# KTH-RPL/HiMo

Hardware: AMD Instinct MI355X
Metric: lidar_frames_per_sec_120k (higher is better)
Workload: dtype f16x2 (two-term split fp16, x = h + l with exact subnormals, on the matrix cores; float32 accumulate; ~22-bit products); 1 GPU; per-frame pipeline: pillarise 3 sweeps (512x512 grid) -> SeFlow++-style encoder/decoder + GRU head (random-init, self-specified: reference network source absent) -> per-point flow -> ego-motion removal + dt0 + flow2compDis -> comp_dis; points_per_frame=120000, sweeps_per_frame=3, parallelism=frames sharded x1, refined_output=False, batches_in_flight=3, matrix_arithmetic=f16x2, samples_per_backbone_launch=16, collectives=none (single process)

## Files before the change

### himo_amd/csrc/gruhead.hip

```cpp
#include "conv_common.h"
#include "bf16x3.h"

namespace himo {

struct GruHeadArgs {
    int64_t n;
    const int* pid; const float* offsets;
    const float* img0; const float* img1; int img_pitch;
    const float* dec; int dec_pitch;
    const float* w_off; const float* b_off;
    const unsigned short* wzr; const float* bzr;
    const unsigned short* wq; const float* bq;
    const unsigned short* w1; const float* b1;
    const float* w2; const float* b2;
    const float* xyz_t; const float* pts; int stride;
    float* flow;
    int iters;
    int img_split;
    unsigned* nonfinite;
    int w2_pitch;
};

constexpr int kGhMaxIters = 4;
struct GruHeadSave {
// ... 8 lines not shown
constexpr int kGhMaxSamples = 16;
struct GruHeadSample {
    int64_t n;
    const int* pid; const float* offsets; const float* img0; const float* img1; const float* dec;
    const float* xyz_t; const float* pts; float* flow; int stride;
};
struct GruHeadBatch {
    int n_samples;
    int block_start[kGhMaxSamples + 1];
    GruHeadSample s[kGhMaxSamples];
};

constexpr int kGhRows = 64;
constexpr bool kGhLaunder = false;

template <int SLABS>
__device__ inline int a_slot(int s, int slab, int row, int half) {
    return ((s * SLABS + slab) * kGhRows + row) * 32 + ((half ^ ((row >> 4) & 1)) << 4);
}

template <int FMT, int SLABS>
__device__ inline void a_store(unsigned char* A, int row, int k, float v) {
    constexpr int kGhPlane = SLABS * kGhRows * 32;
    unsigned h, m = 0, l;
    if (FMT == 3) split3(v, h, m, l); else split2(v, h, l);
    const int slab = k >> 4, kk = k & 15;
    const int off = a_slot<SLABS>(0, slab, row, kk >> 3) + (kk & 7) * 2;
    *reinterpret_cast<unsigned short*>(A + off) = (unsigned short)h;
    if (FMT == 3) *reinterpret_cast<unsigned short*>(A + off + kGhPlane) = (unsigned short)m;
    *reinterpret_cast<unsigned short*>(A + off + (FMT - 1) * kGhPlane) = (unsigned short)l;
// ... 44 lines not shown
#pragma unroll
        for (int rt = 0; rt < RT; ++rt)
#pragma unroll
            for (int t = 0; t < NT; ++t)
#pragma unroll
                for (int r = 0; r < 16; ++r)
                    acc[rt][t][r] = acc[rt][t][r] * kF16AccScale;
    }
}

template <int GROUP>
__device__ inline void sv_store(float* base, unsigned byte_off, float v) {
    *reinterpret_cast<float*>(reinterpret_cast<char*>(base) + byte_off) = v;
}

template <int FMT, int SLABS, bool SAVE = false>
__global__ __launch_bounds__(256, (FMT == 2 && !SAVE) ? 3 : 2) void gru_head_kernel(GruHeadArgs a, GruHeadBatch batch, GruHeadSave sv) {
    constexpr bool FOLD = SLABS == 9;
    static_assert(!(SAVE && FOLD), "the training forward keeps x explicit");
    constexpr int kGhPlane = SLABS * kGhRows * 32;
    __shared__ __attribute__((aligned(16))) unsigned char A[FMT * kGhPlane];
    __shared__ int s_pid[kGhRows];
    const int wave = __builtin_amdgcn_readfirstlane(threadIdx.x >> 6), lane = threadIdx.x & 63;
    const int li = lane & 31, lh = lane >> 5;
    int bid = blockIdx.x;
    {
        int smp = 0;
        while (smp + 1 < batch.n_samples && bid >= batch.block_start[smp + 1]) ++smp;
        bid -= batch.block_start[smp];
        const GruHeadSample& g = batch.s[smp];
        a.n = g.n; a.pid = g.pid; a.offsets = g.offsets; a.img0 = g.img0; a.img1 = g.img1; a.dec = g.dec;
        a.xyz_t = g.xyz_t; a.pts = g.pts; a.flow = g.flow; a.stride = g.stride;
    }
    const int64_t r0 = (int64_t)bid * kGhRows;

    if (threadIdx.x < kGhRows) {
        const int64_t i = r0 + threadIdx.x;
        s_pid[threadIdx.x] = i < a.n ? a.pid[i] : -1;
    }
    if constexpr (FOLD) {
        const int row = threadIdx.x >> 2, q = threadIdx.x & 3;
        const int64_t i = r0 + row;
        float v[4] = {0.f, 0.f, 0.f, 0.f};
        if (q == 0) {
            if (i < a.n) { v[0] = a.offsets[i * 3]; v[1] = a.offsets[i * 3 + 1]; v[2] = a.offsets[i * 3 + 2]; }
            v[3] = 1.f;
        }
// ... 16 lines not shown
        }
    } else {
        const int row = threadIdx.x >> 2, q = threadIdx.x & 3;
        const int64_t i = r0 + row;
        float o0 = 0.f, o1 = 0.f, o2 = 0.f;
        if (i < a.n) { o0 = a.offsets[i * 3]; o1 = a.offsets[i * 3 + 1]; o2 = a.offsets[i * 3 + 2]; }
#pragma unroll
        for (int k = 0; k < 16; ++k) {
            const int c = q * 16 + k;
            const float v = fmaf(o2, a.w_off[128 + c], fmaf(o1, a.w_off[64 + c], o0 * a.w_off[c])) + a.b_off[c];
            a_store<FMT, SLABS>(A, row, 128 + c, v);
        }
    }
    __syncthreads();

    const float* src = wave == 0 ? a.img0 : wave == 1 ? a.img1 : a.dec + (wave - 2) * 32;
    const int src_pitch = wave < 2 ? a.img_pitch : a.dec_pitch;
    float h[2][16];
    {
        int cell[2][16];
#pragma unroll
        for (int rt = 0; rt < 2; ++rt)
#pragma unroll
            for (int r = 0; r < 16; ++r) cell[rt][r] = s_pid[rt * 32 + (r & 3) + 8 * (r >> 2) + 4 * lh];
        if (FMT == 2 && wave < 2 && a.img_split) {
            unsigned short hh[2][16], ll[2][16];
#pragma unroll
            for (int rt = 0; rt < 2; ++rt)
#pragma unroll
                for (int r = 0; r < 16; ++r) {
                    const unsigned short* rec = reinterpret_cast<const unsigned short*>(src + (int64_t)max(cell[rt][r], 0) * src_pitch + (li & ~15));
                    hh[rt][r] = rec[li & 15]; ll[rt][r] = rec[16 + (li & 15)];
                }
#pragma unroll
            for (int rt = 0; rt < 2; ++rt)
#pragma unroll
                for (int r = 0; r < 16; ++r)
                    h[rt][r] = cell[rt][r] >= 0 ? (float)__builtin_bit_cast(_Float16, hh[rt][r]) + (float)__builtin_bit_cast(_Float16, ll[rt][r]) : 0.f;
        } else {
#pragma unroll
// ... 140 lines not shown
            }
            a.flow[i * 3 + c] = out;
            if (a.nonfinite && !(fabsf(out) <= 3.4028234664e38f)) atomicOr(a.nonfinite, 1u);
        }
    }
}

}

using namespace himo;

static int gru_head_launch(int n_samples, const himo_head_sample* h_samples, int img_pitch, int dec_pitch,
                           const float* d_w_off, const float* d_b_off, bool folded,
                           const void* d_wzr_packed, const float* d_bzr, const void* d_wq_packed, const float* d_bq,
                           const void* d_w1_packed, const float* d_b1, const float* d_w2, const float* d_b2,
                           int iters, int packed_format, int img_split, unsigned* d_nonfinite, void* stream) {
    if (img_split && (packed_format != 1 || (img_pitch & 15))) return HIMO_ERR_INVALID_ARGUMENT;
    if (n_samples < 0 || n_samples > kGhMaxSamples || (n_samples && !h_samples)) return HIMO_ERR_INVALID_ARGUMENT;
    if (iters < 0 || !(packed_format == 0 || packed_format == 1) || img_pitch < 32 || dec_pitch < 64) return HIMO_ERR_INVALID_ARGUMENT;
    if ((!folded && (!d_w_off || !d_b_off)) || !d_wzr_packed || !d_bzr || !d_wq_packed || !d_bq || !d_w1_packed || !d_b1 || !d_w2 || !d_b2)
        return HIMO_ERR_INVALID_ARGUMENT;
    if ((reinterpret_cast<uintptr_t>(d_wzr_packed) | reinterpret_cast<uintptr_t>(d_wq_packed) | reinterpret_cast<uintptr_t>(d_w1_packed)) & 15)
        return HIMO_ERR_INVALID_ARGUMENT;
    GruHeadBatch b{};
    int64_t blocks = 0;
    for (int i = 0; i < n_samples; ++i) {
        const himo_head_sample& h = h_samples[i];
        if (h.n < 0 || h.pc_stride < 3) return HIMO_ERR_INVALID_ARGUMENT;
        if (h.n == 0) continue;
        if (!h.d_pid || !h.d_offsets || !h.d_img0 || !h.d_img1 || !h.d_dec || !h.d_xyz_t || !h.d_pts || !h.d_flow) return HIMO_ERR_INVALID_ARGUMENT;
        GruHeadSample& g = b.s[b.n_samples];
        g.n = h.n; g.pid = h.d_pid; g.offsets = h.d_offsets; g.img0 = h.d_img0; g.img1 = h.d_img1; g.dec = h.d_dec;
        g.xyz_t = h.d_xyz_t; g.pts = h.d_pts; g.flow = h.d_flow; g.stride = h.pc_stride;
        b.block_start[b.n_samples] = (int)blocks;
        blocks += (h.n + kGhRows - 1) / kGhRows;
        if (blocks > 0x7fffffff) return HIMO_ERR_INVALID_ARGUMENT;
        b.block_start[++b.n_samples] = (int)blocks;
    }
    if (!blocks) return HIMO_OK;
    GruHeadArgs a{};
    a.img_pitch = img_pitch; a.dec_pitch = dec_pitch; a.w_off = d_w_off; a.b_off = d_b_off;
    a.wzr = (const unsigned short*)d_wzr_packed; a.bzr = d_bzr; a.wq = (const unsigned short*)d_wq_packed; a.bq = d_bq;
    a.w1 = (const unsigned short*)d_w1_packed; a.b1 = d_b1; a.w2 = d_w2; a.b2 = d_b2; a.iters = iters;
    a.img_split = img_split ? 1 : 0;
    a.nonfinite = d_nonfinite;
    a.w2_pitch = 3;
    hipStream_t s = (hipStream_t)stream;
    ProfScope ps("gru_head_kernel", s);
    const dim3 grid((unsigned)blocks);
    const GruHeadSave none{};
    if (folded) {
        if (packed_format == 1) hipLaunchKernelGGL((gru_head_kernel<2, 9>), grid, dim3(256), 0, s, a, b, none);
        else hipLaunchKernelGGL((gru_head_kernel<3, 9>), grid, dim3(256), 0, s, a, b, none);
    } else {
        if (packed_format == 1) hipLaunchKernelGGL((gru_head_kernel<2, 12>), grid, dim3(256), 0, s, a, b, none);
        else hipLaunchKernelGGL((gru_head_kernel<3, 12>), grid, dim3(256), 0, s, a, b, none);
    }
    HIMO_LAUNCH_CHECK("gru_head_kernel");
    return HIMO_OK;
}

extern "C" int himo_gru_head_batch(int n_samples, const himo_head_sample* h_samples, int img_pitch, int dec_pitch,
                                   const float* d_w_off, const float* d_b_off,
                                   const void* d_wzr_packed, const float* d_bzr, const void* d_wq_packed, const float* d_bq,
                                   const void* d_w1_packed, const float* d_b1, const float* d_w2, const float* d_b2,
                                   int iters, int packed_format, int img_split, void* stream) {
    return gru_head_launch(n_samples, h_samples, img_pitch, dec_pitch, d_w_off, d_b_off, false, d_wzr_packed, d_bzr, d_wq_packed, d_bq,
                           d_w1_packed, d_b1, d_w2, d_b2, iters, packed_format, img_split, nullptr, stream);
}

extern "C" int himo_gru_head_batch_folded(int n_samples, const himo_head_sample* h_samples, int img_pitch, int dec_pitch,
                                          const void* d_wzr_packed, const float* d_bzr, const void* d_wq_packed, const float* d_bq,
                                          const void* d_w1_packed, const float* d_b1, const float* d_w2, const float* d_b2,
                                          int iters, int packed_format, int img_split, void* stream) {
    return gru_head_launch(n_samples, h_samples, img_pitch, dec_pitch, nullptr, nullptr, true, d_wzr_packed, d_bzr, d_wq_packed, d_bq,
                           d_w1_packed, d_b1, d_w2, d_b2, iters, packed_format, img_split, nullptr, stream);
}

extern "C" int himo_gru_head_batch_guarded(int n_samples, const himo_head_sample* h_samples, int img_pitch, int dec_pitch,
                                           const float* d_w_off, const float* d_b_off,
                                           const void* d_wzr_packed, const float* d_bzr, const void* d_wq_packed, const float* d_bq,
                                           const void* d_w1_packed, const float* d_b1, const float* d_w2, const float* d_b2,
                                           int iters, int packed_format, int img_split, uint32_t* d_nonfinite, void* stream) {
    if ((d_w_off == nullptr) != (d_b_off == nullptr)) return HIMO_ERR_INVALID_ARGUMENT;
    return gru_head_launch(n_samples, h_samples, img_pitch, dec_pitch, d_w_off, d_b_off, d_w_off == nullptr, d_wzr_packed, d_bzr, d_wq_packed,
                           d_bq, d_w1_packed, d_b1, d_w2, d_b2, iters, packed_format, img_split, d_nonfinite, stream);
}

extern "C" int himo_gru_head_train(int64_t n, const int32_t* d_pid, const float* d_offsets, const float* d_img0, const float* d_img1,
                                   int img_pitch, const float* d_dec, int dec_pitch, const float* d_w_off, const float* d_b_off,
                                   const void* d_wzr_packed, const float* d_bzr, const void* d_wq_packed, const float* d_bq,
                                   const void* d_w1_packed, const float* d_b1, const float* d_w2, int w2_pitch, const float* d_b2,
                                   int iters, int packed_format, const himo_head_saved* h_saved, uint32_t* d_nonfinite, void* stream) {
    if (n < 0 || iters < 1 || iters > kGhMaxIters || !(packed_format == 0 || packed_format == 1) || img_pitch < 32 || dec_pitch < 64 ||
        !(w2_pitch == 3 || w2_pitch == 4) || !h_saved)
        return HIMO_ERR_INVALID_ARGUMENT;
    if (!d_w_off || !d_b_off || !d_wzr_packed || !d_bzr || !d_wq_packed || !d_bq || !d_w1_packed || !d_b1 || !d_w2 || !d_b2)
        return HIMO_ERR_INVALID_ARGUMENT;
    if ((reinterpret_cast<uintptr_t>(d_wzr_packed) | reinterpret_cast<uintptr_t>(d_wq_packed) | reinterpret_cast<uintptr_t>(d_w1_packed)) & 15)
        return HIMO_ERR_INVALID_ARGUMENT;
    if (n == 0) return HIMO_OK;
// ... 7 lines not shown
        return HIMO_ERR_INVALID_ARGUMENT;
    GruHeadBatch b{};
    b.n_samples = 1;
    GruHeadSample& g = b.s[0];
    g.n = n; g.pid = d_pid; g.offsets = d_offsets; g.img0 = d_img0; g.img1 = d_img1; g.dec = d_dec;
    const int64_t blocks = (n + kGhRows - 1) / kGhRows;
    if (blocks > 0x7fffffff) return HIMO_ERR_INVALID_ARGUMENT;
    b.block_start[0] = 0; b.block_start[1] = (int)blocks;
    GruHeadArgs a{};
    a.img_pitch = img_pitch; a.dec_pitch = dec_pitch; a.w_off = d_w_off; a.b_off = d_b_off;
    a.wzr = (const unsigned short*)d_wzr_packed; a.bzr = d_bzr; a.wq = (const unsigned short*)d_wq_packed; a.bq = d_bq;
    a.w1 = (const unsigned short*)d_w1_packed; a.b1 = d_b1; a.w2 = d_w2; a.b2 = d_b2; a.iters = iters; a.w2_pitch = w2_pitch;
    a.nonfinite = d_nonfinite;
    hipStream_t s = (hipStream_t)stream;
    ProfScope ps("gru_head_train_kernel", s);
    if (packed_format == 1) hipLaunchKernelGGL((gru_head_kernel<2, 12, true>), dim3((unsigned)blocks), dim3(256), 0, s, a, b, sv);
    else hipLaunchKernelGGL((gru_head_kernel<3, 12, true>), dim3((unsigned)blocks), dim3(256), 0, s, a, b, sv);
    HIMO_LAUNCH_CHECK("gru_head_kernel<train>");
    return HIMO_OK;
}

extern "C" int himo_clear_u32(uint32_t* d_words, int n, void* stream) {
    if (!d_words || n < 1) return HIMO_ERR_INVALID_ARGUMENT;
    HIMO_HIP(hipMemsetAsync(d_words, 0, (size_t)n * 4, (hipStream_t)stream));
    return HIMO_OK;
}

extern "C" int himo_gru_head(int64_t n, const int32_t* d_pid, const float* d_offsets, const float* d_img0, const float* d_img1,
                             int img_pitch, const float* d_dec, int dec_pitch, const float* d_w_off, const float* d_b_off,
                             const void* d_wzr_packed, const float* d_bzr, const void* d_wq_packed, const float* d_bq,
                             const void* d_w1_packed, const float* d_b1, const float* d_w2, const float* d_b2,
                             const float* d_xyz_t, const float* d_pts, int pc_stride, float* d_flow, int iters, int packed_format,
// ... 6 lines not shown
```

### himo_amd/seflow/model.py

```python
from __future__ import annotations

import ctypes

import numpy as np
import torch

from .. import _lib
from . import spec

EPI_BIAS, EPI_BIAS_BN_GELU, EPI_BIAS_GELU, EPI_GRU_ZR, EPI_GRU_Q = range(5)


class ConvDesc(ctypes.Structure):
    _fields_ = [("x", ctypes.c_void_p), ("x_batch_stride", ctypes.c_int64), ("x_pitch", ctypes.c_int),
                ("w", ctypes.c_void_p), ("bias", ctypes.c_void_p), ("scale", ctypes.c_void_p), ("shift", ctypes.c_void_p),
                ("y", ctypes.c_void_p), ("y_batch_stride", ctypes.c_int64), ("y_pitch", ctypes.c_int),
                ("n", ctypes.c_int), ("h", ctypes.c_int), ("w_in", ctypes.c_int), ("cin", ctypes.c_int),
                ("cout", ctypes.c_int), ("ksize", ctypes.c_int), ("stride", ctypes.c_int), ("epilogue", ctypes.c_int),
                ("aux_in", ctypes.c_void_p), ("aux_in_pitch", ctypes.c_int),
                ("aux_out", ctypes.c_void_p), ("aux_out_pitch", ctypes.c_int), ("w_packed", ctypes.c_void_p),
                ("tile_hint", ctypes.c_int), ("packed_format", ctypes.c_int),
                ("n_outer", ctypes.c_int), ("x_outer_stride", ctypes.c_int64), ("y_outer_stride", ctypes.c_int64),
                ("act_layout", ctypes.c_int), ("range_seen", ctypes.c_void_p)]

# ... 20 lines not shown
                                       ctypes.c_void_p, ctypes.c_int, ctypes.c_void_p]),
    "himo_upsample2x_batch": (ctypes.c_int, [ctypes.c_int, ctypes.c_void_p, ctypes.c_int64, ctypes.c_int, ctypes.c_int, ctypes.c_int,
                                             ctypes.c_int, ctypes.c_void_p, ctypes.c_int64, ctypes.c_int, ctypes.c_void_p]),
    "himo_upsample2x_batch_ex": (ctypes.c_int, [ctypes.c_int, ctypes.c_void_p, ctypes.c_int64, ctypes.c_int, ctypes.c_int, ctypes.c_int,
                                                ctypes.c_int, ctypes.c_void_p, ctypes.c_int64, ctypes.c_int, ctypes.c_int, ctypes.c_void_p]),
    "himo_conv_pack_weights_ex": (ctypes.c_int, [ctypes.c_void_p, ctypes.c_int, ctypes.c_int, ctypes.c_int, ctypes.c_int, ctypes.c_void_p,
                                                 ctypes.c_void_p]),
    "himo_gru_head": (ctypes.c_int, [ctypes.c_int64] + [ctypes.c_void_p] * 4 + [ctypes.c_int, ctypes.c_void_p, ctypes.c_int]
                      + [ctypes.c_void_p] * 12 + [ctypes.c_int, ctypes.c_void_p, ctypes.c_int, ctypes.c_int, ctypes.c_void_p]),
    "himo_gru_head_batch": (ctypes.c_int, [ctypes.c_int, ctypes.c_void_p, ctypes.c_int, ctypes.c_int] + [ctypes.c_void_p] * 10
                            + [ctypes.c_int, ctypes.c_int, ctypes.c_int, ctypes.c_void_p]),
    "himo_gru_head_batch_folded": (ctypes.c_int, [ctypes.c_int, ctypes.c_void_p, ctypes.c_int, ctypes.c_int] + [ctypes.c_void_p] * 8
                                   + [ctypes.c_int, ctypes.c_int, ctypes.c_int, ctypes.c_void_p]),
    "himo_gru_head_batch_guarded": (ctypes.c_int, [ctypes.c_int, ctypes.c_void_p, ctypes.c_int, ctypes.c_int] + [ctypes.c_void_p] * 10
                                    + [ctypes.c_int, ctypes.c_int, ctypes.c_int, ctypes.c_void_p, ctypes.c_void_p]),
    "himo_clear_u32": (ctypes.c_int, [ctypes.c_void_p, ctypes.c_int, ctypes.c_void_p]),
    "himo_head_gather": (ctypes.c_int, [ctypes.c_int64, ctypes.c_void_p, ctypes.c_void_p, ctypes.c_void_p, ctypes.c_void_p,
                                        ctypes.c_int, ctypes.c_void_p, ctypes.c_int, ctypes.c_void_p, ctypes.c_void_p,
                                        ctypes.c_void_p, ctypes.c_void_p, ctypes.c_int, ctypes.c_void_p]),
    "himo_head_final": (ctypes.c_int, [ctypes.c_int64, ctypes.c_void_p, ctypes.c_int, ctypes.c_void_p, ctypes.c_void_p,
                                       ctypes.c_void_p, ctypes.c_void_p, ctypes.c_void_p, ctypes.c_int, ctypes.c_void_p,
                                       ctypes.c_void_p]),
})


class HimoHeadSample(ctypes.Structure):
    _fields_ = [("n", ctypes.c_int64), ("d_pid", ctypes.c_void_p), ("d_offsets", ctypes.c_void_p), ("d_img0", ctypes.c_void_p),
                ("d_img1", ctypes.c_void_p), ("d_dec", ctypes.c_void_p), ("d_xyz_t", ctypes.c_void_p), ("d_pts", ctypes.c_void_p),
                ("pc_stride", ctypes.c_int), ("d_flow", ctypes.c_void_p)]

# ... 53 lines not shown
    def __init__(self, params: dict | None = None, device=None, max_points: int = 140_000, seed: int = 0,
                 precision: str = "bf16x3", autotune: bool = True, max_batch: int = 1):
        if precision not in ("bf16x3", "f16x2", "f32"):
            raise ValueError(precision)
        if max_batch < 1:
            raise ValueError("max_batch")
        self.max_batch = max_batch
        self.precision = precision
        self.autotune = autotune
        self.keep_cell_lists = False
        self.fused_head = precision != "f32"
        self._incremental_images = True
        self.use_plan = True
        self.use_graph = True
        self._plans = {}
        self._recording = None
        self._nb = 1
        self.packed_format = 1 if precision == "f16x2" else 0
        self._split_acts = precision == "f16x2"
        self.tiles = {}
        self.lib = _lib.load()
        self.device = device if device is not None else _lib.require_gpu()
        params = spec.init_params(seed) if params is None else params
        shapes = spec.param_shapes()
        for k, shp in shapes.items():
            if k not in params or tuple(params[k].shape) != tuple(shp):
                raise KeyError(f"parameter {k} missing or of wrong shape (want {shp})")
        cpu = {k: torch.from_numpy(np.ascontiguousarray(params[k], dtype=np.float32)) for k in shapes}
        def fold(prefix, eps):
            scale = cpu[f"{prefix}.gamma"] / torch.sqrt(cpu[f"{prefix}.var"] + eps)
# ... 47 lines not shown
        self.E1 = [buf(F, (H // 2) * (W // 2), 64) for _ in range(2)]
        self.F1 = buf((H // 2) * (W // 2), 64 * F)
        self.E2 = [buf(F, (H // 4) * (W // 4), 128) for _ in range(2)]
        self.F2 = buf((H // 4) * (W // 4), 128 * F)
        self.E3 = [buf(F, (H // 8) * (W // 8), 256) for _ in range(2)]
        self.F3 = buf((H // 8) * (W // 8), 256 * F)
        self.T1 = buf((H // 8) * (W // 8), 256)
        self.CAT1 = buf((H // 4) * (W // 4), 512)
        self.S = [buf((H // 4) * (W // 4), 256) for _ in range(2)]
        self.T2 = buf((H // 4) * (W // 4), 128)
        self.CAT2 = buf((H // 2) * (W // 2), 256)
        self.T = [buf((H // 2) * (W // 2), 128) for _ in range(2)]
        self.T3 = buf((H // 2) * (W // 2), 64)
        self.CAT3 = buf(H * W, 128)
        self.U = [buf(H * W, 64) for _ in range(2)]
        self.DEC = buf(H * W, 64)
        self.max_points = 0
        self._reserve_points(max_points)
        self.guard = torch.zeros(2 + self.MAX_RANGE_SLOTS, dtype=torch.int32, device=dev)
        self.nonfinite = self.guard[:1]
        self._ran_word = self.guard[-1:]
        self._range_slots = {}
        self._range = _f32x(spec.POINT_CLOUD_RANGE[:3])
        self._voxel = _f32x(spec.VOXEL_SIZE)
        r, v = spec.POINT_CLOUD_RANGE, spec.VOXEL_SIZE
        self._centre = _f32x([v[0] / 2 + r[0], v[1] / 2 + r[1], v[2] / 2 + r[2]])

    def _reserve_points(self, n: int):
        if n <= self.max_points:
            return
        dev = self.device
# ... 122 lines not shown
            return cands[0] if cands else 0
        return fastest_tile_hint(self.lib, d, cands, warmup=2)

    def _up(self, x, x_pitch, h, w, c, y, y_pitch, out_split=False):
        nb = self._nb
        osp = 1 if (out_split and self.split_acts) else 0
        if self._recording is not None:
            op = HimoOp(); op.kind = 1
            op.up_x, op.up_x_pitch, op.up_h, op.up_w, op.up_c, op.up_y, op.up_y_pitch = x.data_ptr(), x_pitch, h, w, c, y.data_ptr(), y_pitch
            op.up_n, op.up_x_batch_stride, op.up_y_batch_stride = nb, x.stride(0), y.stride(0)
            op.up_out_split = osp
            self._recording.append(op)
        _lib.check(self.lib.himo_upsample2x_batch_ex(nb, x.data_ptr(), x.stride(0) if nb > 1 else 0, x_pitch, h, w, c, y.data_ptr(),
                                                     y.stride(0) if nb > 1 else 0, y_pitch, osp, _lib.stream_handle()), "himo_upsample2x_batch_ex")

    def backbone(self, n_samples: int = 1):
        if not 1 <= n_samples <= self.max_batch:
            raise ValueError(f"n_samples must be in 1..{self.max_batch}")
        self._nb = n_samples
        if self.packed_format == 1:
            self._ran_word.fill_(1)
        plan = self._plans.get(n_samples)
        if self.use_plan and plan is not None:
            ops, n = plan
            _lib.check(self.lib.himo_run_ops(ctypes.addressof(ops), n, 1 if self.use_graph else 0, _lib.stream_handle()), "himo_run_ops")
            return self.DEC
        self._recording = [] if self.use_plan else None
        self.encoder()
        self.decoder()
        if self._recording is not None:
            rec, self._recording = self._recording, None
            self._plans[n_samples] = ((HimoOp * len(rec))(*rec), len(rec))
        return self.DEC

    def __del__(self):
        try:
            self.drop_plan()
        except Exception:
            pass

    def drop_plan(self):
        for plan in self._plans.values():
            self.lib.himo_ops_release(ctypes.addressof(plan[0]))
        self._plans = {}

    def encoder(self):
        H, W, F = self.H, self.W, self.F
# ... 5 lines not shown
            ho, wo = h // 2, w // 2
            for i in range(n_conv):
                name = f"{stage}.{i}"
                last = i == n_conv - 1
                dst = catbuf if last else pingpong[i % 2]
                dst_bs, dst_pitch = (cout, cout * F) if last else (ho * wo * cout, cout)
                act = ACT_SPLIT_IN | ACT_SPLIT_OUT
                if i == 0:
                    self._conv(src, src_bs, src_pitch, name, dst, dst_bs, dst_pitch, F, h, w, cin, cout, 3, 2,
                               EPI_BIAS_BN_GELU, scale=p[f"{name}.scale"], shift=p[f"{name}.shift"], act=act)
                else:
                    self._conv(src, src_bs, src_pitch, name, dst, dst_bs, dst_pitch, F, ho, wo, cout, cout, 3, 1,
                               EPI_BIAS_BN_GELU, scale=p[f"{name}.scale"], shift=p[f"{name}.shift"], act=act)
                src, src_bs, src_pitch = dst, dst_bs, dst_pitch

    def decoder(self):
        H, W, F = self.H, self.W, self.F
        IN, IO = ACT_SPLIT_IN, ACT_SPLIT_IN | ACT_SPLIT_OUT
        fold = self.fold_decoder
        def block(name, coarse, c_in, ch, cw, tmp, cat, skip, skip_c, lat, out, work, nxt=None):
            if coarse is not None:
                self._conv(coarse, 0, c_in, f"{name}.u1", tmp, 0, lat, 1, 1, ch * cw, c_in, lat, 1, 1, EPI_BIAS, act=IN)
            self._up(tmp, lat, ch, cw, lat, cat, 2 * lat, out_split=True)
            self._conv(skip, 0, skip_c, f"{name}.u3", cat, 0, 2 * lat, 1, 1, 4 * ch * cw, skip_c, lat, 1, 1, EPI_BIAS, y_off=lat, act=IO)
            self._conv(cat, 0, 2 * lat, f"{name}.u4", work[0], 0, out, 1, 2 * ch, 2 * cw, 2 * lat, out, 3, 1, EPI_BIAS, act=IO)
            if fold and nxt is not None:
                nname, ntmp, nlat = nxt
                self._conv(work[0], 0, out, f"{name}.u5>{nname}.u1", ntmp, 0, nlat, 1, 2 * ch, 2 * cw, out, nlat, 3, 1, EPI_BIAS, act=IN)
                return None
            self._conv(work[0], 0, out, f"{name}.u5", work[1], 0, out, 1, 2 * ch, 2 * cw, out, out, 3, 1, EPI_BIAS, act=IO)
            return work[1]
        s = block("dec1", self.F3, 256 * F, H // 8, W // 8, self.T1, self.CAT1, self.F2, 128 * F, 256, 256, self.S, ("dec2", self.T2, 128))
        t = block("dec2", s, 256, H // 4, W // 4, self.T2, self.CAT2, self.F1, 64 * F, 128, 128, self.T, ("dec3", self.T3, 64))
        u = block("dec3", t, 128, H // 2, W // 2, self.T3, self.CAT3, self.B0, 32 * F, 64, 64, self.U)
        self._conv(u, 0, 64, "dec4", self.DEC, 0, 64, 1, H, W, 64, 64, 3, 1, EPI_BIAS, act=IN)
        return self.DEC

    def head(self, pc0: torch.Tensor, slot0: int = 1, slot1: int = 2, out: torch.Tensor | None = None) -> torch.Tensor:
        n = pc0.shape[0]
        p = self.p
        F = self.F
        B0, DEC = self.B0[self._sample], self.DEC[self._sample]
        if self.fused_head:
            flow = out if out is not None else torch.empty((n, 3), dtype=torch.float32, device=self.device)
            if flow.shape != (n, 3) or flow.dtype != torch.float32 or not flow.is_contiguous():
                raise ValueError("out must be a contiguous (N0,3) float32 tensor")
            self.head_batch([pc0], [flow], slot0, slot1, samples=[self._sample])
            return flow
        if self.split_acts:
# ... 30 lines not shown
        T0 = inv1 @ np.asarray(pose0, np.float64)
        Th = inv1 @ np.asarray(pose_h1, np.float64)
        self._use_sample(0)
        self.pillarize_all((pch1, pc0, pc1), (Th, T0, np.eye(4)))
        self.backbone(1)
        return self.head(pc0, out=out)

    def forward_batch(self, samples, outs) -> None:
        if not 1 <= len(samples) <= self.max_batch:
            raise ValueError(f"forward_batch takes 1..{self.max_batch} samples")
        jobs = []
        for k, (pch1, pc0, pc1, pose_h1, pose0, pose1) in enumerate(samples):
            inv1 = np.linalg.inv(np.asarray(pose1, np.float64))
            jobs.append((k, (pch1, pc0, pc1), (inv1 @ np.asarray(pose_h1, np.float64), inv1 @ np.asarray(pose0, np.float64), np.eye(4))))
        self.pillarize_many(jobs)
        self.backbone(len(samples))
        if self.fused_head:
            self.head_batch([smp[1] for smp in samples], outs)
            return
        for k, smp in enumerate(samples):
            self._use_sample(k)
            self.head(smp[1], out=outs[k])

    MAX_HEAD_SAMPLES = 16

    def head_batch(self, pc0s, outs, slot0: int = 1, slot1: int = 2, samples=None) -> None:
        p, pk, F = self.p, self.packed, self.F
        samples = list(range(len(pc0s))) if samples is None else list(samples)
        for lo in range(0, len(pc0s), self.MAX_HEAD_SAMPLES):
            grp = range(lo, min(lo + self.MAX_HEAD_SAMPLES, len(pc0s)))
            arr = (HimoHeadSample * len(grp))()
            for j, i in enumerate(grp):
                k = samples[i]
                pc0, flow, st = pc0s[i], outs[i], self._pt[k]
                n = pc0.shape[0]
                if flow.shape != (n, 3) or flow.dtype != torch.float32 or not flow.is_contiguous():
                    raise ValueError("out must be a contiguous (N0,3) float32 tensor")
                h = arr[j]
                h.n, h.d_pid, h.d_offsets = n, st["pid"][slot0].data_ptr(), st["offsets"][slot0].data_ptr()
                h.d_img0, h.d_img1 = self.B0[k].data_ptr() + 4 * 32 * slot0, self.B0[k].data_ptr() + 4 * 32 * slot1
                h.d_dec, h.d_xyz_t = self.DEC[k].data_ptr(), st["xyz_t"][slot0].data_ptr()
                h.d_pts, h.pc_stride, h.d_flow = pc0.data_ptr(), pc0.shape[1], flow.data_ptr()
            tail = (p["head.dec2.weight"].data_ptr(), p["head.dec2.bias"].data_ptr(),
                    spec.GRU_ITERS, self.packed_format, 1 if self.split_acts else 0, self.nonfinite.data_ptr(), _lib.stream_handle())
            if self.fold_head:
                st = self.lib.himo_gru_head_batch_guarded(len(arr), ctypes.addressof(arr), 32 * F, 64, None, None,
                                                          pk["head.gru.zr.weight.h"].data_ptr(), p["head.gru.zr.bias"].data_ptr(),
                                                          pk["head.gru.q.weight.h"].data_ptr(), p["head.gru.q.bias"].data_ptr(),
                                                          pk["head.dec1.weight.h"].data_ptr(), p["head.dec1.bias"].data_ptr(), *tail)
            else:
                st = self.lib.himo_gru_head_batch_guarded(len(arr), ctypes.addressof(arr), 32 * F, 64,
                                                          p["head.offset.weight"].data_ptr(), p["head.offset.bias"].data_ptr(),
                                                          pk["head.gru.zr.weight"].data_ptr(), p["head.gru.zr.bias"].data_ptr(),
                                                          pk["head.gru.q.weight"].data_ptr(), p["head.gru.q.bias"].data_ptr(),
                                                          pk["head.dec1.weight"].data_ptr(), p["head.dec1.bias"].data_ptr(), *tail)
            _lib.check(st, "himo_gru_head_batch")

    def pillarize_all(self, sweeps, transforms):
        self.pillarize_many([(self._sample, sweeps, transforms)])

# ... 98 lines not shown
```

### include/himo_amd.h

```cpp
#ifndef HIMO_AMD_H
#define HIMO_AMD_H

#include <stddef.h>
#include <stdint.h>

#ifdef __cplusplus
extern "C" {
#endif

#define HIMO_ABI_VERSION 1

typedef enum himo_status {
    HIMO_OK = 0,
    HIMO_ERR_INVALID_ARGUMENT = 1,
    HIMO_ERR_EMPTY_FRAME = 2,
    HIMO_ERR_WORKSPACE = 3,
    HIMO_ERR_SINGULAR_POSE = 4,
    HIMO_ERR_HIP = 5,
    HIMO_ERR_UNSUPPORTED = 6
} himo_status;

#define HIMO_FLAG_F32_CHAIN 0x1u
#define HIMO_FLAG_RAW 0x2u
#define HIMO_FLAG_SCANIA 0x4u
// ... 292 lines not shown
} himo_head_sample;
int himo_gru_head_batch(int n_samples, const himo_head_sample* h_samples, int img_pitch, int dec_pitch,
                        const float* d_w_off, const float* d_b_off,
                        const void* d_wzr_packed, const float* d_bzr, const void* d_wq_packed, const float* d_bq,
                        const void* d_w1_packed, const float* d_b1, const float* d_w2, const float* d_b2,
                        int iters, int packed_format, int img_split, void* stream);
int himo_gru_head_batch_folded(int n_samples, const himo_head_sample* h_samples, int img_pitch, int dec_pitch,
                               const void* d_wzr_packed, const float* d_bzr, const void* d_wq_packed, const float* d_bq,
                               const void* d_w1_packed, const float* d_b1, const float* d_w2, const float* d_b2,
                               int iters, int packed_format, int img_split, void* stream);
int himo_gru_head_batch_guarded(int n_samples, const himo_head_sample* h_samples, int img_pitch, int dec_pitch,
                                const float* d_w_off, const float* d_b_off,
                                const void* d_wzr_packed, const float* d_bzr, const void* d_wq_packed, const float* d_bq,
                                const void* d_w1_packed, const float* d_b1, const float* d_w2, const float* d_b2,
                                int iters, int packed_format, int img_split, uint32_t* d_nonfinite, void* stream);
typedef struct himo_head_saved {
    int64_t rows;
    float* d_hx;
    float* d_rhx;
    float* d_z; float* d_r; float* d_q;
    float* d_pre1; float* d_y1;
    float* d_res;
} himo_head_saved;
int himo_gru_head_train(int64_t n, const int32_t* d_pid, const float* d_offsets, const float* d_img0, const float* d_img1,
                        int img_pitch, const float* d_dec, int dec_pitch, const float* d_w_off, const float* d_b_off,
                        const void* d_wzr_packed, const float* d_bzr, const void* d_wq_packed, const float* d_bq,
                        const void* d_w1_packed, const float* d_b1, const float* d_w2, int w2_pitch, const float* d_b2,
                        int iters, int packed_format, const himo_head_saved* h_saved, uint32_t* d_nonfinite, void* stream);
int himo_gru_head_backward(int64_t n, int iters, const float* d_dhx_last, const himo_head_saved* h_saved,
                           const void* d_wq_t_packed, const void* d_wzr_t_packed, int packed_format, float* d_daq,
// ... 218 lines not shown
```

Measured before the change: 747.1 frames/s.

## Fuse decoder's last conv into GRU head, evaluated only at point cells

Drops the dense final decoder 3x3 conv (dec4) over the full 512x512 grid from the backbone plan. The head kernel instead computes that conv for each point's cell only, doing a 9-tap MFMA gather over the U[1] map with a software-pipelined load of weights and activations. This avoids a full-grid conv and the DEC write and re-read. In exchange the head does redundant work when several points share a cell, adds register pressure to the head kernel, and leaves DEC stale on this path.

```diff
diff --git a/himo_amd/csrc/gruhead.hip b/himo_amd/csrc/gruhead.hip
--- a/himo_amd/csrc/gruhead.hip
+++ b/himo_amd/csrc/gruhead.hip
@@ -46,6 +46,65 @@
 constexpr int kGhRows = 64;
 constexpr bool kGhLaunder = false;
 
+struct GruHeadDec4 {
+    const unsigned char* map[kGhMaxSamples];
+    const unsigned char* w; const float* bias;
+    int pitch_bytes, W, H;
+};
+__device__ __attribute__((aligned(256))) unsigned char g_gh_zero_rec[256];
+
+__device__ inline void dec4_rows(const GruHeadDec4& d, const unsigned char* __restrict__ map, const int* s_pid, int ct, int li, int lh,
+                                 floatx16 (&acc)[2]) {
+    const unsigned char* ap[2][9];
+#pragma unroll
+    for (int rt = 0; rt < 2; ++rt) {
+        const int pid = s_pid[rt * 32 + li];
+        const int y = pid / d.W, x = pid - y * d.W;
+#pragma unroll
+        for (int t = 0; t < 9; ++t) {
+            const int ny = y + t / 3 - 1, nx = x + t % 3 - 1;
+            const bool ok = pid >= 0 && ny >= 0 && ny < d.H && nx >= 0 && nx < d.W;
+            ap[rt][t] = (ok ? map + ((int64_t)ny * d.W + nx) * d.pitch_bytes : g_gh_zero_rec) + lh * 16;
+        }
+    }
+    const unsigned char* __restrict__ wb = d.w;
+    const unsigned b_lane = (unsigned)(ct * 32 + li) * 32u + (unsigned)lh * 16u;
+    constexpr unsigned b_plane = 64u * 32u, b_block = 2u * b_plane;
+    uint4 bq[3][2];
+    f16x8 aq[3][2][2];
+#define HIMO_DEC4_LOAD(TAP, SLAB, SET)                                                                             \
+    do {                                                                                                           \
+        const unsigned off = (unsigned)((TAP) * 4 + (SLAB)) * b_block + b_lane;                                    \
+        bq[SET][0] = *reinterpret_cast<const uint4*>(wb + off);                                                    \
+        bq[SET][1] = *reinterpret_cast<const uint4*>(wb + (off + b_plane));                                        \
+        _Pragma("unroll") for (int rt = 0; rt < 2; ++rt) _Pragma("unroll") for (int s = 0; s < 2; ++s)              \
+            aq[SET][rt][s] = *reinterpret_cast<const f16x8*>(ap[rt][TAP] + ((SLAB) * 64 + s * 32));                 \
+    } while (0)
+#pragma unroll
+    for (int rt = 0; rt < 2; ++rt)
+#pragma unroll
+        for (int r = 0; r < 16; ++r) acc[rt][r] = 0.f;
+    HIMO_DEC4_LOAD(0, 0, 0);
+    HIMO_DEC4_LOAD(1, 0, 1);
+#pragma unroll 1
+    for (int slab = 0; slab < 4; ++slab) {
+        const int nslab = slab < 3 ? slab + 1 : slab;
+#pragma unroll
+        for (int tap = 0; tap < 9; ++tap) {
+            if (tap + 2 < 9) HIMO_DEC4_LOAD(tap + 2, slab, (tap + 2) % 3);
+            else HIMO_DEC4_LOAD(tap + 2 - 9, nslab, (tap + 2) % 3);
+#define HIMO_TERM16(SA, SB)                                                                                        \
+    _Pragma("unroll") for (int rt = 0; rt < 2; ++rt)                                                                 \
+        acc[rt] = __builtin_amdgcn_mfma_f32_32x32x16_f16(aq[tap % 3][rt][SA], __builtin_bit_cast(f16x8, bq[tap % 3][SB]), acc[rt], 0, 0, 0);
+            HIMO_TERM16(1, 0) HIMO_TERM16(0, 1) HIMO_TERM16(0, 0)
+#undef HIMO_TERM16
+            __builtin_amdgcn_sched_group_barrier(0x020, 6, 0);
+            __builtin_amdgcn_sched_group_barrier(0x008, 6, 0);
+        }
+    }
+#undef HIMO_DEC4_LOAD
+}
+
 template <int SLABS>
 __device__ inline int a_slot(int s, int slab, int row, int half) {
     return ((s * SLABS + slab) * kGhRows + row) * 32 + ((half ^ ((row >> 4) & 1)) << 4);
@@ -120,10 +179,12 @@
     *reinterpret_cast<float*>(reinterpret_cast<char*>(base) + byte_off) = v;
 }
 
-template <int FMT, int SLABS, bool SAVE = false>
-__global__ __launch_bounds__(256, (FMT == 2 && !SAVE) ? 3 : 2) void gru_head_kernel(GruHeadArgs a, GruHeadBatch batch, GruHeadSave sv) {
+template <int FMT, int SLABS, bool SAVE = false, bool DEC4 = false>
+__global__ __launch_bounds__(256, (FMT == 2 && !SAVE) ? 3 : 2) void gru_head_kernel(GruHeadArgs a, GruHeadBatch batch, GruHeadSave sv, GruHeadDec4 d4) {
     constexpr bool FOLD = SLABS == 9;
     static_assert(!(SAVE && FOLD), "the training forward keeps x explicit");
+    static_assert(!DEC4 || (FMT == 2 && FOLD && !SAVE), "the decoder's last layer is fused into the folded fp16-split inference head only");
+    const unsigned char* d4_map = nullptr;
     constexpr int kGhPlane = SLABS * kGhRows * 32;
     __shared__ __attribute__((aligned(16))) unsigned char A[FMT * kGhPlane];
     __shared__ int s_pid[kGhRows];
@@ -137,6 +198,7 @@
         const GruHeadSample& g = batch.s[smp];
         a.n = g.n; a.pid = g.pid; a.offsets = g.offsets; a.img0 = g.img0; a.img1 = g.img1; a.dec = g.dec;
         a.xyz_t = g.xyz_t; a.pts = g.pts; a.flow = g.flow; a.stride = g.stride;
+        if constexpr (DEC4) d4_map = d4.map[smp];
     }
     const int64_t r0 = (int64_t)bid * kGhRows;
 
@@ -183,7 +245,7 @@
     }
     __syncthreads();
 
-    const float* src = wave == 0 ? a.img0 : wave == 1 ? a.img1 : a.dec + (wave - 2) * 32;
+    const float* src = wave == 0 ? a.img0 : wave == 1 ? a.img1 : DEC4 ? nullptr : a.dec + (wave - 2) * 32;
     const int src_pitch = wave < 2 ? a.img_pitch : a.dec_pitch;
     float h[2][16];
     {
@@ -192,7 +254,19 @@
         for (int rt = 0; rt < 2; ++rt)
 #pragma unroll
             for (int r = 0; r < 16; ++r) cell[rt][r] = s_pid[rt * 32 + (r & 3) + 8 * (r >> 2) + 4 * lh];
-        if (FMT == 2 && wave < 2 && a.img_split) {
+        if (DEC4 && wave >= 2) {
+            if constexpr (DEC4) {
+                floatx16 acd[2];
+                dec4_rows(d4, d4_map, s_pid, wave - 2, li, lh, acd);
+                float eA, eB;
+                epi_affine<kEpiBias>(kF16AccScale, d4.bias[(wave - 2) * 32 + li], 1.f, 0.f, eA, eB);
+#pragma unroll
+                for (int rt = 0; rt < 2; ++rt)
+#pragma unroll
+                    for (int r = 0; r < 16; ++r)
+                        h[rt][r] = s_pid[rt * 32 + (r & 3) + 8 * (r >> 2) + 4 * lh] >= 0 ? epi_activate<kEpiBias>(acd[rt][r], eA, eB) : 0.f;
+            }
+        } else if (FMT == 2 && wave < 2 && (DEC4 || a.img_split)) {
             unsigned short hh[2][16], ll[2][16];
 #pragma unroll
             for (int rt = 0; rt < 2; ++rt)
@@ -363,7 +437,8 @@
                            const float* d_w_off, const float* d_b_off, bool folded,
                            const void* d_wzr_packed, const float* d_bzr, const void* d_wq_packed, const float* d_bq,
                            const void* d_w1_packed, const float* d_b1, const float* d_w2, const float* d_b2,
-                           int iters, int packed_format, int img_split, unsigned* d_nonfinite, void* stream) {
+                           int iters, int packed_format, int img_split, unsigned* d_nonfinite, void* stream,
+                           const GruHeadDec4* dec4 = nullptr, const float* const* h_maps = nullptr) {
     if (img_split && (packed_format != 1 || (img_pitch & 15))) return HIMO_ERR_INVALID_ARGUMENT;
     if (n_samples < 0 || n_samples > kGhMaxSamples || (n_samples && !h_samples)) return HIMO_ERR_INVALID_ARGUMENT;
     if (iters < 0 || !(packed_format == 0 || packed_format == 1) || img_pitch < 32 || dec_pitch < 64) return HIMO_ERR_INVALID_ARGUMENT;
@@ -372,12 +447,18 @@
     if ((reinterpret_cast<uintptr_t>(d_wzr_packed) | reinterpret_cast<uintptr_t>(d_wq_packed) | reinterpret_cast<uintptr_t>(d_w1_packed)) & 15)
         return HIMO_ERR_INVALID_ARGUMENT;
     GruHeadBatch b{};
+    GruHeadDec4 d4{};
+    if (dec4) d4 = *dec4;
     int64_t blocks = 0;
     for (int i = 0; i < n_samples; ++i) {
         const himo_head_sample& h = h_samples[i];
         if (h.n < 0 || h.pc_stride < 3) return HIMO_ERR_INVALID_ARGUMENT;
         if (h.n == 0) continue;
-        if (!h.d_pid || !h.d_offsets || !h.d_img0 || !h.d_img1 || !h.d_dec || !h.d_xyz_t || !h.d_pts || !h.d_flow) return HIMO_ERR_INVALID_ARGUMENT;
+        if (!h.d_pid || !h.d_offsets || !h.d_img0 || !h.d_img1 || (!dec4 && !h.d_dec) || !h.d_xyz_t || !h.d_pts || !h.d_flow) return HIMO_ERR_INVALID_ARGUMENT;
+        if (dec4) {
+            if (!h_maps[i] || (reinterpret_cast<uintptr_t>(h_maps[i]) & 15)) return HIMO_ERR_INVALID_ARGUMENT;
+            d4.map[b.n_samples] = reinterpret_cast<const unsigned char*>(h_maps[i]);
+        }
         GruHeadSample& g = b.s[b.n_samples];
         g.n = h.n; g.pid = h.d_pid; g.offsets = h.d_offsets; g.img0 = h.d_img0; g.img1 = h.d_img1; g.dec = h.d_dec;
         g.xyz_t = h.d_xyz_t; g.pts = h.d_pts; g.flow = h.d_flow; g.stride = h.pc_stride;
@@ -398,12 +479,14 @@
     ProfScope ps("gru_head_kernel", s);
     const dim3 grid((unsigned)blocks);
     const GruHeadSave none{};
-    if (folded) {
-        if (packed_format == 1) hipLaunchKernelGGL((gru_head_kernel<2, 9>), grid, dim3(256), 0, s, a, b, none);
-        else hipLaunchKernelGGL((gru_head_kernel<3, 9>), grid, dim3(256), 0, s, a, b, none);
+    if (dec4) {
+        hipLaunchKernelGGL((gru_head_kernel<2, 9, false, true>), grid, dim3(256), 0, s, a, b, none, d4);
+    } else if (folded) {
+        if (packed_format == 1) hipLaunchKernelGGL((gru_head_kernel<2, 9>), grid, dim3(256), 0, s, a, b, none, d4);
+        else hipLaunchKernelGGL((gru_head_kernel<3, 9>), grid, dim3(256), 0, s, a, b, none, d4);
     } else {
-        if (packed_format == 1) hipLaunchKernelGGL((gru_head_kernel<2, 12>), grid, dim3(256), 0, s, a, b, none);
-        else hipLaunchKernelGGL((gru_head_kernel<3, 12>), grid, dim3(256), 0, s, a, b, none);
+        if (packed_format == 1) hipLaunchKernelGGL((gru_head_kernel<2, 12>), grid, dim3(256), 0, s, a, b, none, d4);
+        else hipLaunchKernelGGL((gru_head_kernel<3, 12>), grid, dim3(256), 0, s, a, b, none, d4);
     }
     HIMO_LAUNCH_CHECK("gru_head_kernel");
     return HIMO_OK;
@@ -434,6 +517,24 @@
     if ((d_w_off == nullptr) != (d_b_off == nullptr)) return HIMO_ERR_INVALID_ARGUMENT;
     return gru_head_launch(n_samples, h_samples, img_pitch, dec_pitch, d_w_off, d_b_off, d_w_off == nullptr, d_wzr_packed, d_bzr, d_wq_packed,
                            d_bq, d_w1_packed, d_b1, d_w2, d_b2, iters, packed_format, img_split, d_nonfinite, stream);
+}
+
+extern "C" int himo_gru_head_batch_dec4(int n_samples, const himo_head_sample* h_samples, const float* const* h_maps, int img_pitch,
+                                        int map_pitch, int grid_w, int grid_h, const void* d_wdec4_packed, const float* d_bdec4,
+                                        const float* d_w_off, const float* d_b_off,
+                                        const void* d_wzr_packed, const float* d_bzr, const void* d_wq_packed, const float* d_bq,
+                                        const void* d_w1_packed, const float* d_b1, const float* d_w2, const float* d_b2,
+                                        int iters, int packed_format, int img_split, uint32_t* d_nonfinite, void* stream) {
+    if (d_w_off || d_b_off) return HIMO_ERR_INVALID_ARGUMENT;
+    if (packed_format != 1 || !img_split) return HIMO_ERR_INVALID_ARGUMENT;
+    if (!d_wdec4_packed || !d_bdec4 || (reinterpret_cast<uintptr_t>(d_wdec4_packed) & 15) || (n_samples > 0 && !h_maps)) return HIMO_ERR_INVALID_ARGUMENT;
+    if (map_pitch < 64 || (map_pitch & 15) || grid_w < 1 || grid_h < 1) return HIMO_ERR_INVALID_ARGUMENT;
+    if ((int64_t)grid_w * grid_h * map_pitch * 4 >= ((int64_t)1 << 31)) return HIMO_ERR_INVALID_ARGUMENT;
+    GruHeadDec4 d4{};
+    d4.w = reinterpret_cast<const unsigned char*>(d_wdec4_packed); d4.bias = d_bdec4;
+    d4.pitch_bytes = map_pitch * 4; d4.W = grid_w; d4.H = grid_h;
+    return gru_head_launch(n_samples, h_samples, img_pitch, 64, nullptr, nullptr, true, d_wzr_packed, d_bzr, d_wq_packed, d_bq,
+                           d_w1_packed, d_b1, d_w2, d_b2, iters, packed_format, img_split, d_nonfinite, stream, &d4, h_maps);
 }
 
 extern "C" int himo_gru_head_train(int64_t n, const int32_t* d_pid, const float* d_offsets, const float* d_img0, const float* d_img1,
@@ -471,8 +572,9 @@
     a.nonfinite = d_nonfinite;
     hipStream_t s = (hipStream_t)stream;
     ProfScope ps("gru_head_train_kernel", s);
-    if (packed_format == 1) hipLaunchKernelGGL((gru_head_kernel<2, 12, true>), dim3((unsigned)blocks), dim3(256), 0, s, a, b, sv);
-    else hipLaunchKernelGGL((gru_head_kernel<3, 12, true>), dim3((unsigned)blocks), dim3(256), 0, s, a, b, sv);
+    const GruHeadDec4 no_dec4{};
+    if (packed_format == 1) hipLaunchKernelGGL((gru_head_kernel<2, 12, true>), dim3((unsigned)blocks), dim3(256), 0, s, a, b, sv, no_dec4);
+    else hipLaunchKernelGGL((gru_head_kernel<3, 12, true>), dim3((unsigned)blocks), dim3(256), 0, s, a, b, sv, no_dec4);
     HIMO_LAUNCH_CHECK("gru_head_kernel<train>");
     return HIMO_OK;
 }
diff --git a/himo_amd/seflow/model.py b/himo_amd/seflow/model.py
--- a/himo_amd/seflow/model.py
+++ b/himo_amd/seflow/model.py
@@ -58,6 +58,8 @@
                                    + [ctypes.c_int, ctypes.c_int, ctypes.c_int, ctypes.c_void_p]),
     "himo_gru_head_batch_guarded": (ctypes.c_int, [ctypes.c_int, ctypes.c_void_p, ctypes.c_int, ctypes.c_int] + [ctypes.c_void_p] * 10
                                     + [ctypes.c_int, ctypes.c_int, ctypes.c_int, ctypes.c_void_p, ctypes.c_void_p]),
+    "himo_gru_head_batch_dec4": (ctypes.c_int, [ctypes.c_int, ctypes.c_void_p, ctypes.c_void_p] + [ctypes.c_int] * 4 + [ctypes.c_void_p] * 12
+                                 + [ctypes.c_int, ctypes.c_int, ctypes.c_int, ctypes.c_void_p, ctypes.c_void_p]),
     "himo_clear_u32": (ctypes.c_int, [ctypes.c_void_p, ctypes.c_int, ctypes.c_void_p]),
     "himo_head_gather": (ctypes.c_int, [ctypes.c_int64, ctypes.c_void_p, ctypes.c_void_p, ctypes.c_void_p, ctypes.c_void_p,
                                         ctypes.c_int, ctypes.c_void_p, ctypes.c_int, ctypes.c_void_p, ctypes.c_void_p,
@@ -141,6 +143,11 @@
         self.use_plan = True
         self.use_graph = True
         self._plans = {}
+        self.fuse_dec4 = True
+        """``forward_batch`` under precision "f16x2" with ``split_acts``, ``fused_head`` and ``fold_head``: the decoder's last
+        layer (dec4) runs inside the head kernel, at the cells of the points only (himo_gru_head_batch_dec4), and the backbone plan
+        stops at its input ``U[1]``.  ``DEC`` is NOT produced on that path (it keeps what the last dense pass left; zeros at first).
+        Same flow bits either way; False -- and every other configuration or entry point -- keeps the dense layer."""
         self._recording = None
         self._nb = 1
         self.packed_format = 1 if precision == "f16x2" else 0
@@ -218,7 +225,7 @@
         self.T3 = buf((H // 2) * (W // 2), 64)
         self.CAT3 = buf(H * W, 128)
         self.U = [buf(H * W, 64) for _ in range(2)]
-        self.DEC = buf(H * W, 64)
+        self.DEC = torch.zeros((B, H * W, 64), dtype=torch.float32, device=dev)
         self.max_points = 0
         self._reserve_points(max_points)
         self.guard = torch.zeros(2 + self.MAX_RANGE_SLOTS, dtype=torch.int32, device=dev)
@@ -371,23 +378,23 @@
         _lib.check(self.lib.himo_upsample2x_batch_ex(nb, x.data_ptr(), x.stride(0) if nb > 1 else 0, x_pitch, h, w, c, y.data_ptr(),
                                                      y.stride(0) if nb > 1 else 0, y_pitch, osp, _lib.stream_handle()), "himo_upsample2x_batch_ex")
 
-    def backbone(self, n_samples: int = 1):
+    def backbone(self, n_samples: int = 1, without_dec4: bool = False):
         if not 1 <= n_samples <= self.max_batch:
             raise ValueError(f"n_samples must be in 1..{self.max_batch}")
         self._nb = n_samples
         if self.packed_format == 1:
             self._ran_word.fill_(1)
-        plan = self._plans.get(n_samples)
+        plan = self._plans.get((n_samples, without_dec4))
         if self.use_plan and plan is not None:
             ops, n = plan
             _lib.check(self.lib.himo_run_ops(ctypes.addressof(ops), n, 1 if self.use_graph else 0, _lib.stream_handle()), "himo_run_ops")
             return self.DEC
         self._recording = [] if self.use_plan else None
         self.encoder()
-        self.decoder()
+        self.decoder(without_dec4)
         if self._recording is not None:
             rec, self._recording = self._recording, None
-            self._plans[n_samples] = ((HimoOp * len(rec))(*rec), len(rec))
+            self._plans[(n_samples, without_dec4)] = ((HimoOp * len(rec))(*rec), len(rec))
         return self.DEC
 
     def __del__(self):
@@ -423,7 +430,7 @@
                                EPI_BIAS_BN_GELU, scale=p[f"{name}.scale"], shift=p[f"{name}.shift"], act=act)
                 src, src_bs, src_pitch = dst, dst_bs, dst_pitch
 
-    def decoder(self):
+    def decoder(self, without_dec4: bool = False):
         H, W, F = self.H, self.W, self.F
         IN, IO = ACT_SPLIT_IN, ACT_SPLIT_IN | ACT_SPLIT_OUT
         fold = self.fold_decoder
@@ -442,6 +449,8 @@
         s = block("dec1", self.F3, 256 * F, H // 8, W // 8, self.T1, self.CAT1, self.F2, 128 * F, 256, 256, self.S, ("dec2", self.T2, 128))
         t = block("dec2", s, 256, H // 4, W // 4, self.T2, self.CAT2, self.F1, 64 * F, 128, 128, self.T, ("dec3", self.T3, 64))
         u = block("dec3", t, 128, H // 2, W // 2, self.T3, self.CAT3, self.B0, 32 * F, 64, 64, self.U)
+        if without_dec4:
+            return u
         self._conv(u, 0, 64, "dec4", self.DEC, 0, 64, 1, H, W, 64, 64, 3, 1, EPI_BIAS, act=IN)
         return self.DEC
 
@@ -502,9 +511,10 @@
             inv1 = np.linalg.inv(np.asarray(pose1, np.float64))
             jobs.append((k, (pch1, pc0, pc1), (inv1 @ np.asarray(pose_h1, np.float64), inv1 @ np.asarray(pose0, np.float64), np.eye(4))))
         self.pillarize_many(jobs)
-        self.backbone(len(samples))
+        fuse = bool(self.fuse_dec4 and self.packed_format == 1 and self.split_acts and self.fused_head and self.fold_head)
+        self.backbone(len(samples), without_dec4=fuse)
         if self.fused_head:
-            self.head_batch([smp[1] for smp in samples], outs)
+            self.head_batch([smp[1] for smp in samples], outs, dec4_fused=fuse)
             return
         for k, smp in enumerate(samples):
             self._use_sample(k)
@@ -512,12 +522,13 @@
 
     MAX_HEAD_SAMPLES = 16
 
-    def head_batch(self, pc0s, outs, slot0: int = 1, slot1: int = 2, samples=None) -> None:
+    def head_batch(self, pc0s, outs, slot0: int = 1, slot1: int = 2, samples=None, dec4_fused: bool = False) -> None:
         p, pk, F = self.p, self.packed, self.F
         samples = list(range(len(pc0s))) if samples is None else list(samples)
         for lo in range(0, len(pc0s), self.MAX_HEAD_SAMPLES):
             grp = range(lo, min(lo + self.MAX_HEAD_SAMPLES, len(pc0s)))
             arr = (HimoHeadSample * len(grp))()
+            maps = (ctypes.c_void_p * len(grp))()
             for j, i in enumerate(grp):
                 k = samples[i]
                 pc0, flow, st = pc0s[i], outs[i], self._pt[k]
@@ -528,10 +539,17 @@
                 h.n, h.d_pid, h.d_offsets = n, st["pid"][slot0].data_ptr(), st["offsets"][slot0].data_ptr()
                 h.d_img0, h.d_img1 = self.B0[k].data_ptr() + 4 * 32 * slot0, self.B0[k].data_ptr() + 4 * 32 * slot1
                 h.d_dec, h.d_xyz_t = self.DEC[k].data_ptr(), st["xyz_t"][slot0].data_ptr()
+                maps[j] = self.U[1][k].data_ptr()
                 h.d_pts, h.pc_stride, h.d_flow = pc0.data_ptr(), pc0.shape[1], flow.data_ptr()
             tail = (p["head.dec2.weight"].data_ptr(), p["head.dec2.bias"].data_ptr(),
                     spec.GRU_ITERS, self.packed_format, 1 if self.split_acts else 0, self.nonfinite.data_ptr(), _lib.stream_handle())
-            if self.fold_head:
+            if dec4_fused:
+                st = self.lib.himo_gru_head_batch_dec4(len(arr), ctypes.addressof(arr), ctypes.addressof(maps), 32 * F, 64, self.W, self.H,
+                                                       pk["dec4.weight"].data_ptr(), p["dec4.bias"].data_ptr(), None, None,
+                                                       pk["head.gru.zr.weight.h"].data_ptr(), p["head.gru.zr.bias"].data_ptr(),
+                                                       pk["head.gru.q.weight.h"].data_ptr(), p["head.gru.q.bias"].data_ptr(),
+                                                       pk["head.dec1.weight.h"].data_ptr(), p["head.dec1.bias"].data_ptr(), *tail)
+            elif self.fold_head:
                 st = self.lib.himo_gru_head_batch_guarded(len(arr), ctypes.addressof(arr), 32 * F, 64, None, None,
                                                           pk["head.gru.zr.weight.h"].data_ptr(), p["head.gru.zr.bias"].data_ptr(),
                                                           pk["head.gru.q.weight.h"].data_ptr(), p["head.gru.q.bias"].data_ptr(),
diff --git a/include/himo_amd.h b/include/himo_amd.h
--- a/include/himo_amd.h
+++ b/include/himo_amd.h
@@ -330,6 +330,12 @@
                                 const void* d_wzr_packed, const float* d_bzr, const void* d_wq_packed, const float* d_bq,
                                 const void* d_w1_packed, const float* d_b1, const float* d_w2, const float* d_b2,
                                 int iters, int packed_format, int img_split, uint32_t* d_nonfinite, void* stream);
+int himo_gru_head_batch_dec4(int n_samples, const himo_head_sample* h_samples, const float* const* h_maps, int img_pitch,
+                             int map_pitch, int grid_w, int grid_h, const void* d_wdec4_packed, const float* d_bdec4,
+                             const float* d_w_off, const float* d_b_off,
+                             const void* d_wzr_packed, const float* d_bzr, const void* d_wq_packed, const float* d_bq,
+                             const void* d_w1_packed, const float* d_b1, const float* d_w2, const float* d_b2,
+                             int iters, int packed_format, int img_split, uint32_t* d_nonfinite, void* stream);
 typedef struct himo_head_saved {
     int64_t rows;
     float* d_hx;
```

Result: no change. 745.1 frames/s (-0.3%).
